# lxvm/AutoBZCore.jl

Hardware: AMD Instinct MI355X
Metric: k-point evals/sec (H(k)+eig) (higher is better)
Workload: dtype f64

## Files before the change

### autobzcore.jl_amd/_lib.py

```python
import ctypes as C
import os

import numpy as np

_HERE = os.path.dirname(os.path.abspath(__file__))
LIB_PATH = os.environ.get("ABZ_LIB") or os.path.join(_HERE, "libabzhip.so")

c_i32p = C.POINTER(C.c_int32)
c_i64p = C.POINTER(C.c_int64)
c_f64p = C.POINTER(C.c_double)
c_vpp = C.POINTER(C.c_void_p)
c_ip = C.POINTER(C.c_int)

PROTOTYPES = {
    "abz_last_error": (C.c_char_p, []),
    "abz_version": (C.c_int, []),
    "abz_device_count": (C.c_int, [c_ip]),
    "abz_ctx_create": (C.c_int, [C.c_int, c_vpp]),
    "abz_ctx_create_on_stream": (C.c_int, [C.c_int, C.c_void_p, c_vpp]),
    "abz_ctx_destroy": (C.c_int, [C.c_void_p]),
    "abz_ctx_sync": (C.c_int, [C.c_void_p]),
    "abz_prof_enable": (C.c_int, [C.c_void_p, C.c_int]),
    "abz_prof_reset": (C.c_int, [C.c_void_p]),
    "abz_prof_read": (C.c_int, [C.c_void_p, C.c_int, c_f64p, c_i64p]),
# ... 41 lines not shown
    "abz_rule_ltm_node_weights_ptr": (C.c_int, [C.c_void_p, c_vpp, c_i64p, c_ip]),
    "abz_rule_ltm_node_weights_dot": (C.c_int, [C.c_void_p, c_f64p]),
    "abz_rule_ltm_node_weights_fold": (C.c_int, [C.c_void_p, c_f64p]),
    "abz_rule_ltm_density_matrix": (C.c_int, [C.c_void_p, c_f64p]),
    "abz_rule_ltm_green_node_weights": (C.c_int, [C.c_void_p, c_f64p, C.c_int, c_f64p]),
    "abz_rule_ltm_green_node_weights_ptr": (C.c_int, [C.c_void_p, c_vpp, c_i64p, c_ip]),
    "abz_rule_ltm_green_node_weights_dot": (C.c_int, [C.c_void_p, c_f64p]),
    "abz_rule_ltm_green_node_weights_fold": (C.c_int, [C.c_void_p, c_f64p]),
    "abz_rule_ltm_green_node_weights_matrix": (C.c_int, [C.c_void_p, c_f64p]),
    "abz_mem_info": (C.c_int, [C.c_void_p, c_i64p]),
    "abz_symptr_rule": (C.c_int, [C.c_int, C.c_int, c_i32p, C.c_int, c_i64p, c_i32p, c_i64p]),
    "abz_symptr_rule_device": (C.c_int, [C.c_void_p, C.c_int, C.c_int, c_i32p, C.c_int, c_i64p, c_i32p, c_i64p]),
    "abz_contract_nodes": (C.c_int, [C.c_void_p, C.c_int, c_i64p, c_f64p, C.c_int64, c_i64p]),
    "abz_eval_line_nodes": (C.c_int, [C.c_void_p, c_i64p, c_f64p, c_f64p, C.c_int64, C.c_int, c_f64p, C.c_int,
                                      C.c_double, c_f64p]),
    "abz_release_level": (C.c_int, [C.c_void_p, C.c_int]),
    "abz_iai_solve": (C.c_int, [C.c_void_p, C.c_int, c_f64p, c_f64p, C.c_int, c_f64p, C.c_int, C.c_double, C.c_double,
                                C.c_double, C.c_int64, C.c_int64, c_f64p, c_f64p, c_i64p, c_f64p, C.c_int64, c_i64p]),
    "abz_iai_solve_many": (C.c_int, [C.c_void_p, C.c_int, c_f64p, c_f64p, C.c_int, c_f64p, C.c_int, c_f64p, C.c_int,
                                     C.c_double, C.c_double, C.c_int64, C.c_int64, c_f64p, c_f64p, c_i64p, c_f64p,
                                     C.c_int64, c_i64p]),
    "abz_iai_set_exchange": (C.c_int, [C.c_void_p, C.c_void_p, C.c_void_p, C.c_int, C.c_int]),
    "abz_gk15_nodes": (C.c_int, [C.c_double, C.c_double, c_f64p]),
    "abz_gk15_batch": (C.c_int, [c_f64p, c_f64p, C.c_int64, C.c_int, c_f64p, c_f64p]),
}

WANT_H, WANT_EIG, WANT_VEL = 1, 2, 4
WANT_H_COMPACT = 8
WANT_H_ROW_MAJOR = 16
F_ONE, F_LINEAR, F_LINEAR_X, F_DOS, F_TRGLOC, F_GLOC, F_DOS_EIG = range(7)
LIMS_CUBIC, LIMS_TETRAHEDRAL, LIMS_POLYHEDRAL, LIMS_POLYGON = 0, 1, 2, 3
K_CONTRACT, K_EVAL, K_REDUCE, K_GGR, K_EIG, K_GGRBUILD, K_LTM = range(7)
K_EVAL_FUSED = 7
LTM_DOS, LTM_STATES, LTM_STATES_CORRECTED = 0, 1, 2
LTM_A_ELEMENTS, LTM_A_ENERGY = 0, 1
LTM_A_ONE = 2
LTM_MAX_COMP = 16
LTM_EXPECT_MAX_OPS = 8
LTM_PAIRS_MAX_OPS = 4
MAX_BANDS = 64
LTM_NODEW_MAX_E = 16
LTM_GREEN_NODEW_MAX_Z = 8
PIVOT_NONE, PIVOT_PARTIAL = 0, 1
ERR_ARG, ERR_HIP, ERR_NOGPU, ERR_UNSUPPORTED, ERR_NOMEM, ERR_INTERNAL = -1, -2, -3, -4, -5, -6


EXCHANGE_FN = C.CFUNCTYPE(C.c_int, C.c_void_p, C.POINTER(C.c_double), C.c_int64)


class AbzError(RuntimeError):
    """A libabzhip call failed (ABZ_ERR_ARG is raised as ValueError = the reference's ArgumentError)."""


_lib = None


def lib():
    global _lib
    if _lib is None:
        if not os.path.exists(LIB_PATH):
            raise AbzError(f"{LIB_PATH} is missing: build it with __graft_entry__.build(); "
                           "the product has no CPU fallback")
        handle = C.CDLL(LIB_PATH)
        for name, (res, args) in PROTOTYPES.items():
            fn = getattr(handle, name)
            fn.restype = res
# ... 78 lines not shown
```

### autobzcore.jl_amd/csrc/abz_internal.h

```cpp
#pragma once
#include <hip/hip_ext.h>
#include <hip/hip_runtime.h>

#include <atomic>
#include <cstdint>
#include <cstdio>
#include <memory>
#include <string>
#include <vector>

#include "../../include/abzhip.h"
#include "dev_buf.h"
#include "ltm_block.h"
#include "plane_view.h"

namespace abz {
struct ProfScope;
struct RulePlan;

void set_error(const char* fmt, ...);
int catch_status() noexcept;

#define ABZ_CATCH_ALL \
    catch (...) { return abz::catch_status(); }
// ... 19 lines not shown
enum Switch {
    SW_POOL_MB,
    SW_DEBUG_TIMING,
    SW_EVAL_PACKED,
    SW_DOS3_SCAN,
    SW_REDUCE_ROWS,
    SW_ADAPT_PAIR,
    SW_GEN_SUM_TRI,
    SW_IPANEL_FOLD,
    SW_IPANEL_FMAC,
    SW_GGR_FUSED,
    SW_GGR_FUSE2,
    SW_GGR_UNIFORM,
    SW_IAI_SPECULATE,
    SW_IAI_PACKED,
    SW_IAI_POOL_MB,
    SW_IAI_DEVICE_INNER,
    SW_IAI_PANELS,
    SW_IAI_STATS,
    SW_HOST_THREADS,
    SW_AUTO_SWEEP_MAPPED,
    SW_LANE_KERNELS,
    SW_BIG_MFMA,
    SW_BIG_CHUNK_MB,
    SW_BIG_TRI_WAVES,
    SW_EIG_FOLD,
    SW_EIG_SPLIT,
    SW_IAI_LANES,
    SW_IAI_LANE_MIN,
    SW_CHAIN_FUSED,
    SW_EVAL_FUSED,
    SW_EVAL_PAIRS,
    SW_EVAL_MIRROR,
    SW_COUNT
};
int abz_switch(Switch s);

int stage_h2d(abz_ctx* ctx, void* dst_dev, const void* src_host, size_t bytes);
int stage_d2h(abz_ctx* ctx, void* dst_host, const void* src_dev, size_t bytes);
int mbox_reserve(abz_ctx* ctx);

int sweep_to_device(abz_ctx* ctx, const double* host, int n, const double** dev);

struct SumOut {
    double* host = nullptr;
    double* dev = nullptr;
    double2* map_dev = nullptr;
    const double2* map_host = nullptr;
};
int sum_target(abz_ctx* ctx, const SumOut& so, int64_t col0, int64_t ncols, double2** where);
int sum_deliver(abz_ctx* ctx, const SumOut& so, const double2* from, int64_t col0, int64_t ncols);

struct EnergyList {
    std::vector<int> perm;
    std::vector<double> Es, res;
    const double* dev = nullptr;
    double* out = nullptr;
    double* extra = nullptr;
    const double* res_host = nullptr;
    bool mbox = false;
    int width = 1;
    double inv_step = 0.0;
};
int energies_to_device(abz_ctx* ctx, const double* Es_host, int n, bool uniform, size_t extra, EnergyList& el, int width = 1);
int energies_deliver(abz_ctx* ctx, EnergyList& el, double* out_host);
struct SymTables;
int sym_tables_device(abz_ctx* ctx, int npt, int d, const int32_t* syms, int nsyms, SymTables& out);
void preload_symptr_code();

struct SymTables {
    int npt = 0, d = 0;
    int64_t nk = 0;
    int64_t nitems[ABZ_MAX_DIM + 1] = {0, 0, 0, 0};
    DevBuf arena;
    size_t arena_bytes = 0;
    int32_t* idx = nullptr;
    double* w = nullptr;
    int32_t* gi[ABZ_MAX_DIM + 1] = {nullptr, nullptr, nullptr, nullptr};
    int64_t* parent[ABZ_MAX_DIM + 1] = {nullptr, nullptr, nullptr, nullptr};
    int64_t* runs = nullptr;
    std::vector<int32_t> syms;
};

struct ProfSlot {
    double ms = 0.0;
    int64_t launches = 0;
    std::vector<std::pair<hipEvent_t, hipEvent_t>> pending;
};

}

struct abz_ctx {
    std::atomic<int> refs{1};
    bool closed = false;
    int device = 0;
    hipStream_t stream = nullptr;
    bool owns_stream = true;
    unsigned prof = 0;
    abz::ProfScope* prof_scope = nullptr;
    abz::ProfSlot prof_slots[ABZ_K_COUNT];
    std::vector<hipEvent_t> event_pool;
    abz::DevBuf scratch[8];
    void* pin = nullptr;
    size_t pin_cap = 0;
    std::vector<std::unique_ptr<abz::SymTables>> sym_cache;
    std::vector<std::pair<int, abz::DevBuf>> phase_cache;
    void* mbox = nullptr;
    void* mbox_dev = nullptr;
    size_t mbox_cap = 0;
};

namespace abz {
inline bool mbox_half_fits(abz_ctx* ctx, size_t bytes) { return mbox_reserve(ctx) == ABZ_OK && bytes <= ctx->mbox_cap / 2; }
template <class T>
inline T* mbox_results(abz_ctx* ctx, bool device_view) {
    return reinterpret_cast<T*>(static_cast<char*>(device_view ? ctx->mbox_dev : ctx->mbox) + ctx->mbox_cap / 2);
}
inline SumOut sum_out_mailbox(abz_ctx* ctx, double* host, size_t ncols) {
    SumOut so;
    so.host = host;
    if (mbox_half_fits(ctx, sizeof(double2) * ncols)) {
        so.map_dev = mbox_results<double2>(ctx, true);
        so.map_host = mbox_results<const double2>(ctx, false);
    }
    return so;
}
struct SeriesRule {
    int npt = 0, want = 0;
    std::vector<int32_t> syms;
    abz_rule* r = nullptr;
    uint64_t generation = 0;
    uint64_t stamp = 0;
};
// ... 130 lines not shown
int launch_contract(abz_ctx* ctx, const double2* src, int64_t src_slot_elems, const int64_t* parents,
                    int64_t per_parent, const double2* phs, double2* out, int64_t B, int64_t L, int M);

constexpr int ABZ_CONTRACT_GRID_MAXM = 16;
int launch_contract_grid(abz_ctx* ctx, const double2* src, int64_t src_slot_elems, int64_t nparents, const double2* tab,
                         double2* out, int64_t L, int M, int first, int npt, bool deriv, int gbeg, int gcnt,
                         const double2* phs_table = nullptr);
bool contract_chain_fits(int64_t L, int M3, int M2, int npt, int gcnt);
int launch_contract_chain(abz_ctx* ctx, const double2* src, const double2* phs3, const double2* phs2, double2* out,
                          int64_t L, int M3, int M2, int npt, int gbeg, int gcnt);

struct EvalSpec {
    int n;
    int M, first;
    double period;
    const double2* src;
    bool grid;
    int npt;
    int64_t nlines;
    const double2* tab;
    int64_t nk;
    const int64_t* run_start = nullptr;
    int64_t nruns = 0;
    const int64_t* parents;
    const int32_t* gi;
    const double* x;
    bool deriv;
    bool herm;
    bool packed = false;
    const double2* src2 = nullptr;
    const double2* phs2 = nullptr;
    int M2 = 0;
    bool mirror = false;
    PlaneView H;
    PlaneView E;
    PlaneView U;
};
int launch_eval(abz_ctx* ctx, const EvalSpec& es);
bool eval_packed_supported(int n, int M, int npt);
bool eval_mirror_supported(const EvalSpec& es);
bool eval_fused_supported(int n, int64_t mnn, int M2, int npt, bool pairs = false);
int launch_pack_rows(abz_ctx* ctx, int n, int M, const double2* src, int64_t nrows, double2* out);
size_t packed_row_elems(int n, int M);
int series_ensure_packed(abz_series* s);

int launch_eig_planes(abz_ctx* ctx, int n, PlaneView H, PlaneView E, PlaneView U, int64_t nk);
int launch_velocity(abz_ctx* ctx, int n, PlaneView U, PlaneView dH, PlaneView Vj, int64_t nk);

struct ReduceSpec {
    int n, d, npt;
    int integrand;
    PlaneView H;
    PlaneView E;
    int64_t nk;
    const double* w;
    const int32_t* idx;
    int64_t k_offset = 0;
    bool herm = false;
    bool pivot = false;
    double params[4];
    const double* sweep_dev;
    int n_sweep;
    double scale;
    double* tri_cache = nullptr;
    int64_t tri_nk = 0;
    int* tri_state = nullptr;
// ... 240 lines not shown
```

### autobzcore.jl_amd/csrc/api.cpp

```cpp
#include <algorithm>
#include <atomic>
#include <cstdarg>
#include <chrono>
#include <cmath>
#include <cstring>
#include <map>
#include <mutex>
#include <numeric>
#include <thread>

#include "abz_internal.h"

namespace abz {

static thread_local std::string g_err;

void set_error(const char* fmt, ...) {
    char buf[1024];
    va_list ap;
    va_start(ap, fmt);
    vsnprintf(buf, sizeof(buf), fmt, ap);
    va_end(ap);
    g_err = buf;
}
// ... 31 lines not shown
const SwitchDef g_switches[SW_COUNT] = {
    {"ABZ_POOL_MB", 4096, "MB of freed device blocks the caching allocator keeps per device"},
    {"ABZ_DEBUG_TIMING", 0, "1: wall time of the rule-build phases on stderr (synchronises after each)"},
    {"ABZ_EVAL_PACKED", 1, "0: full-grid chains on plain coefficient sets instead of packed Hermitian sets"},
    {"ABZ_DOS3_SCAN", 1, "0: 3-band DOS sweeps through the generic reduce_kernel"},
    {"ABZ_REDUCE_ROWS", 0, "> 0: rows of blocks a sweep is split over in the scan kernels"},
    {"ABZ_ADAPT_PAIR", 1, "0: one-lane adaptive step in the device-side GK loops"},
    {"ABZ_GEN_SUM_TRI", 1, "0: 5...16-band sweeps with one inversion per swept value"},
    {"ABZ_IPANEL_FOLD", 1, "0: 16-lane panel kernel on the unfolded series"},
    {"ABZ_IPANEL_FMAC", 1, "0: 16-lane panel kernel with separate pivot-row broadcasts"},
    {"ABZ_GGR_FUSED", 1, "0: GGR build by eigenvectors + one velocity launch per variable"},
    {"ABZ_GGR_FUSE2", 1, "0: fused GGR build reads level-1 families instead of contracting variable 2 itself"},
    {"ABZ_GGR_UNIFORM", 1, "0: GGR scans search the energy window even in equispaced lists"},
    {"ABZ_IAI_SPECULATE", 1, "0: nested IAI driver requests one panel per integral and round"},
    {"ABZ_IAI_PACKED", 1, "0: IAI chains on plain coefficient sets"},
    {"ABZ_IAI_POOL_MB", 0, "> 0: MB per chunk of level sets in the IAI driver (default: sized from free memory)"},
    {"ABZ_IAI_DEVICE_INNER", 1, "0: innermost GK loops driven from the host, one launch per round"},
    {"ABZ_IAI_PANELS", 1, "0: the level above the innermost one ships nodes instead of panels (GK rule of that level on the host)"},
    {"ABZ_IAI_STATS", 0, "1: per-solve statistics of the IAI driver on stderr"},
    {"ABZ_HOST_THREADS", 8, "host threads for the per-integral bookkeeping of IAI sweeps (capped at half the cores)"},
    {"ABZ_AUTO_SWEEP_MAPPED", 1, "0: abz_autoptr_solve* uploads its swept values instead of letting the kernels read the pinned host copy"},
    {"ABZ_LANE_KERNELS", 1, "0: 5...8-band rule builds / store-free sums on full grids through the 8-lane row kernels (test: same values)"},
    {"ABZ_BIG_MFMA", 0, "1: 33...64 bands: the level-1 evaluation of full grid lines as a real GEMM on v_mfma_f64_16x16x4_f64 (test: same values)"},
    {"ABZ_BIG_CHUNK_MB", 0, "33...64 bands: MB of scratch for the matrices of a chunk of nodes (0: 256, GGR builds 2048; tests set 1 to walk many chunks)"},
    {"ABZ_BIG_TRI_WAVES", 0, "33...64 bands: waves per node of the Householder tridiagonalisation (1, 2, 4: the same reflectors, another summation order; 0: two up to 44 bands, one up to 48, four above)"},
    {"ABZ_EIG_FOLD", 1, "0: 5...16-band rule builds evaluate the full level-1 series of a Hermitian model instead of the folded one"},
    {"ABZ_EIG_SPLIT", 1, "0: eigenvalues of 5...16-band rules by bisection inside the grid kernel instead of the per-lane QR kernel"},
    {"ABZ_IAI_LANES", 4, "lanes (host thread + stream each) a sweep of independent IAI solves is split over; 1: off"},
    {"ABZ_IAI_LANE_MIN", 16, "solves per lane below which a sweep is not split further"},
    {"ABZ_CHAIN_FUSED", 1, "0: 3-D full-grid chains contract variables 3 and 2 in two launches instead of contract_chain_kernel"},
    {"ABZ_EVAL_FUSED", 1, "0: 3-D full-grid rules (n <= 4) build level-1 sets with contract_chain_kernel instead of contracting variable 2 inside the grid kernel"},
    {"ABZ_EVAL_PAIRS", 1, "fused grid kernel, one grid line per half-wave: 1 where it takes fewer lane-rounds per line (Hermitian series), 0 never, 2 wherever supported (tests: same values)"},
    {"ABZ_EVAL_MIRROR", 1, "3-D full-grid rules (n <= 4) of a real Hermitian series evaluate the planes k3 <= npt/2 and store H(-k) = conj H(k) beside them: 1 where the launch writes at most 600 MB, 0 never (every plane evaluated), 2 wherever supported"},
};
}

int abz_switch(Switch s) {
    const char* e = getenv(g_switches[s].name);
    return (e && *e) ? atoi(e) : g_switches[s].dflt;
}

namespace {
struct Block {
    void* p;
    size_t cap;
    int device;
};
std::mutex g_pool_mutex;
std::vector<Block> g_pool;
size_t g_pool_bytes = 0;
std::atomic<int64_t> g_live_bytes{0};
std::atomic<int64_t> g_live_blocks{0};
size_t pool_limit() {
    static const size_t lim = (size_t)std::max(0, abz_switch(SW_POOL_MB)) << 20;
    return lim;
}
void pool_flush(int device) {
    for (size_t i = 0; i < g_pool.size();) {
        if (g_pool[i].device == device) {
            (void)hipFree(g_pool[i].p);
            g_pool_bytes -= g_pool[i].cap;
            g_pool[i] = g_pool.back();
            g_pool.pop_back();
        } else {
            ++i;
        }
// ... 244 lines not shown
}

ProfScope::ProfScope(abz_ctx* c, int kernel_id) : ctx(c), id(kernel_id) {
    if (!(ctx->prof & (1u << id))) return;
    auto get = [&]() {
        hipEvent_t e = nullptr;
        if (!ctx->event_pool.empty()) {
            e = ctx->event_pool.back();
            ctx->event_pool.pop_back();
        } else if (hipEventCreateWithFlags(&e, hipEventDisableSystemFence) != hipSuccess) {
            e = nullptr;
        }
        return e;
    };
    e0 = get();
    e1 = get();
    if (!e0 || !e1) return;
    outer = ctx->prof_scope;
    ctx->prof_scope = this;
}

ProfScope::~ProfScope() {
    if (!(ctx->prof & (1u << id))) return;
    if (e0 && e1) ctx->prof_scope = outer;
    if (!e0 || !e1 || !started) {
        if (e0) ctx->event_pool.push_back(e0);
        if (e1) ctx->event_pool.push_back(e1);
        return;
    }
    ctx->prof_slots[id].pending.emplace_back(e0, e1);
}

int prof_collect(abz_ctx* ctx) {
    for (int i = 0; i < ABZ_K_COUNT; ++i) {
        auto& sl = ctx->prof_slots[i];
        for (auto& pr : sl.pending) {
            ABZ_HIP(hipEventSynchronize(pr.second));
            float ms = 0.f;
            ABZ_HIP(hipEventElapsedTime(&ms, pr.first, pr.second));
            sl.ms += ms;
            sl.launches += 1;
            ctx->event_pool.push_back(pr.first);
            ctx->event_pool.push_back(pr.second);
        }
        sl.pending.clear();
    }
    return ABZ_OK;
}

template <class T>
static int upload(abz_ctx* ctx, DevBuf& buf, const T* host, size_t count) {
    int rc = buf.reserve(sizeof(T) * std::max<size_t>(count, 1));
    if (rc) return rc;
    if (count) return stage_h2d(ctx, buf.p, host, sizeof(T) * count);
    return ABZ_OK;
}

struct Plan {
    int d = 0;
    bool full = false;
    bool coords = false;
    int npt = 0;
    int outer0 = 0, outer_n = 0;
    int64_t nk = 0;
    int64_t nitems[ABZ_MAX_DIM + 1] = {0, 0, 0, 0};
    std::vector<int32_t> gi[ABZ_MAX_DIM + 1];
    std::vector<double> xs[ABZ_MAX_DIM + 1];
// ... 333 lines not shown
    ABZ_REQUIRE(ctx, "null ctx");
    ctx->prof = on == 0 ? 0u : (on == 1 ? 0xffffffffu : ((unsigned)on >> 1));
    return ABZ_OK;
} ABZ_CATCH_ALL

int abz_mem_info(abz_ctx* ctx, int64_t* info) try {
    ABZ_REQUIRE(info, "abz_mem_info: null info");
    {
        std::lock_guard<std::mutex> lk(g_pool_mutex);
        info[1] = (int64_t)g_pool_bytes;
    }
    info[0] = g_live_bytes.load();
    info[2] = 0;
    info[3] = 0;
    info[4] = g_live_blocks.load();
    if (ctx) {
        for (const auto& b : ctx->scratch) info[2] += (int64_t)b.cap;
        info[3] = (int64_t)ctx->pin_cap;
    }
    return ABZ_OK;
} ABZ_CATCH_ALL

int abz_prof_reset(abz_ctx* ctx) try {
    ABZ_REQUIRE(ctx, "null ctx");
    int rc = prof_collect(ctx);
    for (auto& sl : ctx->prof_slots) {
        sl.ms = 0;
        sl.launches = 0;
    }
    return rc;
} ABZ_CATCH_ALL

int abz_prof_read(abz_ctx* ctx, int kernel_id, double* total_ms, int64_t* launches) try {
    ABZ_REQUIRE(ctx && kernel_id >= 0 && kernel_id < ABZ_K_COUNT, "bad profile slot");
    int rc = prof_collect(ctx);
    if (rc) return rc;
    if (total_ms) *total_ms = ctx->prof_slots[kernel_id].ms;
    if (launches) *launches = ctx->prof_slots[kernel_id].launches;
    return ABZ_OK;
} ABZ_CATCH_ALL

static bool detect_hermitian(const abz_series* s, const double* coef_reim);
static bool detect_real(const abz_series* s, const double* coef_reim);

int abz_series_create(abz_ctx* ctx, const double* coef_reim, int d, const int32_t* dims, const int32_t* first,
                      const double* period, int n, abz_series** out) try {
    ABZ_REQUIRE(ctx && coef_reim && dims && first && period && out, "abz_series_create: null argument");
    ABZ_REQUIRE(!ctx->closed, "abz_series_create: the context was destroyed");
    ABZ_REQUIRE(d >= 1 && d <= ABZ_MAX_DIM, "series dimension d = %d not in 1..%d", d, ABZ_MAX_DIM);
    ABZ_REQUIRE(n >= 1 && n <= ABZ_MAX_BANDS, "n = %d bands not in 1..%d", n, ABZ_MAX_BANDS);
    *out = nullptr;
    ABZ_HIP(hipSetDevice(ctx->device));
    std::unique_ptr<abz_series> s(new abz_series());
    s->ctx = ctx;
    s->d = d;
    s->n = n;
    for (int j = 0; j < d; ++j) {
        ABZ_REQUIRE(dims[j] >= 1 && period[j] > 0, "dims[%d] = %d / period = %g invalid", j, dims[j], period[j]);
        s->dims[j] = dims[j];
        s->first[j] = first[j];
        s->period[j] = period[j];
    }
    const size_t bytes = sizeof(double2) * (size_t)s->elems(d);
    if (s->coef.alloc(bytes)) return ABZ_ERR_NOMEM;
    hipError_t e = hipMemcpy(s->coef.p, coef_reim, bytes, hipMemcpyHostToDevice);
    if (e != hipSuccess) {
        set_error("coefficient upload failed: %s", hipGetErrorString(e));
// ... 293 lines not shown
                        const double2* level2 = nullptr) -> int {
        EvalSpec es;
        es.n = n;
        es.M = s->dims[0];
        es.first = s->first[0];
        es.period = s->period[0];
        es.src = level1;
        if (level2) {
            es.src2 = level2;
            es.phs2 = rp->pd.phg[1].as<double2>();
            es.M2 = s->dims[1];
        }
        es.grid = r->full;
        es.npt = r->npt;
        es.nlines = r->full ? (d == 1 ? 1 : plan.nitems[1]) : 0;
        es.tab = tab;
        es.nk = r->nk;
        es.parents = r->full ? nullptr : rp->pd.parent[0].as<int64_t>();
        es.gi = r->full ? nullptr : rp->pd.gi[0].as<int32_t>();
        if (!r->full && plan.nruns > 0 && !plan.coords) {
            es.run_start = rp->pd.runs.as<int64_t>();
            es.nruns = plan.nruns;
        }
        es.x = nullptr;
        es.deriv = deriv;
        es.herm = s->hermitian;
        es.packed = packed_chain && !deriv && !Uout.base;
        const int sw_mirror = abz_switch(SW_EVAL_MIRROR);
        const PlaneView& pv = Hout.base ? Hout : Eout;
        const double out_bytes = 8.0 * ((Hout.base ? (Hout.compact ? 1.0 : 2.0) * n * n : 0.0) + (Eout.base ? (double)n : 0.0)) *
                                 (double)pv.row * (double)es.nlines;
        es.mirror = s->hermitian && s->real_coef && r->full && d == 3 && plan.outer_n == r->npt && !deriv && !Uout.base &&
                    !(r->want & ABZ_WANT_VEL) && (sw_mirror >= 2 || (sw_mirror == 1 && out_bytes <= 600e6));
        es.H = Hout;
        es.E = Eout;
        es.U = Uout;
        return launch_eval(ctx, es);
    };
    const double2* level1 = nullptr;
    int rc;
    const int64_t line_elems = packed_chain ? (int64_t)packed_row_elems(n, s->dims[0]) : (int64_t)s->dims[0] * n * n;
    const bool ref_layout_large = s->hermitian && r->H.base && !r->H.compact && r->npt > 64;
    const bool eval_fused = r->full && d == 3 && n <= 4 && !(r->want & ABZ_WANT_VEL) && !Uv.base && rp->pd.phg[2].p && rp->pd.phg[1].p &&
                            !ref_layout_large &&
                            abz_switch(SW_CHAIN_FUSED) && abz_switch(SW_EVAL_FUSED) &&
                            contract_chain_fits(line_elems, s->dims[2], s->dims[1], r->npt, plan.outer_n) &&
                            eval_fused_supported(n, line_elems, s->dims[1], r->npt);
    if (eval_fused) {
        const double2* level2 = nullptr;
        if ((rc = build_chain(s, plan, rp->pd, tab, 0, &level2, 2, nullptr, packed_chain))) return rc;
        return run_eval(nullptr, false, r->H, r->E, PlaneView(), level2);
    }
    if ((rc = build_chain(s, plan, rp->pd, tab, 0, &level1, 1, nullptr, packed_chain))) return rc;
    if ((rc = run_eval(level1, false, r->H, vel_done ? PlaneView() : r->E, Uv))) return rc;
    if ((r->want & ABZ_WANT_VEL) && !vel_done) {
        for (int j = 1; j <= d; ++j) {
            if (j >= 2)
                if ((rc = build_chain(s, plan, rp->pd, tab, j, &level1))) return rc;
            if ((rc = run_eval(level1, j == 1, Dv, PlaneView(), PlaneView()))) return rc;
            PlaneView Vj = r->V;
            Vj.base += (int64_t)(j - 1) * n * Vj.pitch;
            if ((rc = launch_velocity(ctx, n, Uv, Dv, Vj, r->nk))) return rc;
        }
    }
    return ABZ_OK;
}
// ... 876 lines not shown
```

### autobzcore.jl_amd/csrc/kernels.hip

```cpp
#include "abz_internal.h"
#include "device_math.h"
#include "gk15.h"
#include "inner_adapt.h"
#include "packed_herm.h"

#include <cmath>
#include <cstring>
#include <type_traits>
#include <utility>
#include <cstdlib>

namespace abz {

static inline int64_t cdiv(int64_t a, int64_t b) { return (a + b - 1) / b; }

struct cplx_pod {
    double x, y;
};
typedef const cplx_pod __attribute__((address_space(4))) * cptr_t;
__device__ __forceinline__ cptr_t as_const(const double2* p) {
    return (cptr_t)(unsigned long long)p;
}

struct PhaseArgs {
// ... 771 lines not shown
__device__ __forceinline__ void load_line_phases(cptr_t p, LinePhases& ph) {
#pragma unroll
    for (int m = 0; m < ABZ_CONTRACT_GRID_MAXM; ++m) {
        ph.x[m] = p[m].x;
        ph.y[m] = p[m].y;
    }
}

template <int M2>
__device__ __forceinline__ void contract_line(const double2* s2, const LinePhases& ph, double2* dst, int MNN, int lane) {
    for (int l = lane; l < MNN; l += 64) {
        double ar = 0.0, ai = 0.0;
#pragma unroll
        for (int m = 0; m < M2; ++m) {
            const double2 c = s2[m * MNN + l];
            ar = fma(c.x, ph.x[m], ar);
            ar = fma(-c.y, ph.y[m], ar);
            ai = fma(c.x, ph.y[m], ai);
            ai = fma(c.y, ph.x[m], ai);
        }
        dst[l] = make_double2(ar, ai);
    }
}

__device__ __forceinline__ void contract_line_m(int M2, const double2* s2, const LinePhases& ph, double2* dst, int MNN, int lane) {
#define CL(MM) case MM: contract_line<MM>(s2, ph, dst, MNN, lane); break;
    switch (M2) {
        CL(1) CL(2) CL(3) CL(4) CL(5) CL(6) CL(7) CL(8) CL(9) CL(10) CL(11) CL(12) CL(13) CL(14) CL(15) CL(16)
        default: break;
    }
#undef CL
}

template <int N, int KPL, bool HERM, bool VEC, int OCC, bool PK = false, bool FUSE = false, bool PAIR = false, int KT = KPL, bool MIR = false>
__global__ __launch_bounds__(256, OCC) void eval_grid_kernel(EvalArgs a) {
    static_assert(!MIR || (HERM && !VEC), "mirrored launches: values and eigenvalues of a Hermitian series");
    static_assert(FUSE || !PAIR, "the pair mapping exists in the fused instance only");
    static_assert(KT >= 1 && KT <= KPL && (PAIR || KT == KPL), "a shorter last pass exists in the pair mapping only");
    constexpr int LPU = PAIR ? 2 : 1;
    extern __shared__ double2 lds_c[];
    const int wave = __builtin_amdgcn_readfirstlane(threadIdx.x >> 6), lane = threadIdx.x & 63;
    const int MNN = PK ? Pk<N>::size((a.M - 1) / 2) : a.M * N * N;
    auto stage = [&](double2 c, int idx) -> double2 {
        if (!a.deriv) return c;
        const double f = 6.283185307179586476925286766559 * (double)(a.first + idx / (N * N));
        return make_double2(-f * c.y, f * c.x);
    };
    double2* const mybuf = lds_c + (size_t)wave * 2 * LPU * MNN;
    int fm = a.first % a.npt;
    if (fm < 0) fm += a.npt;
    constexpr int LW = 64 / LPU;
    const int npass = (a.npt + LW * KPL - 1) / (LW * KPL);
    double2* const tab_l = lds_c + (size_t)4 * 2 * LPU * MNN;
    if constexpr (FUSE) {
        static_assert(!VEC, "the fused instance stores values and eigenvalues only");
        const int k3 = blockIdx.y, seg = blockIdx.x;
        const int mk3 = (MIR && k3 != 0 && 2 * k3 != a.npt) ? a.npt - k3 : -1;
        const int L2 = a.M2 * MNN;
        const double2* __restrict__ src2 = a.src2 + (int64_t)k3 * L2;
        double2* const s2 = tab_l + a.npt;
        const int kstride = 4 * a.bpk;
        int k2 = LPU * (4 * seg + wave);
        LinePhases ph;
        load_line_phases(as_const(a.phs2 + (int64_t)(k2 < a.npt ? k2 : 0) * a.M2), ph);
        {
            const int it = threadIdx.x;
            double2 vt = a.tab[min(it, a.npt - 1)];
            double2 v[4];
#pragma unroll
            for (int j = 0; j < 4; ++j) v[j] = src2[min(it + 256 * j, L2 - 1)];
            asm volatile("" : "+v"(vt.x), "+v"(vt.y));
#pragma unroll
            for (int j = 0; j < 4; ++j) asm volatile("" : "+v"(v[j].x), "+v"(v[j].y));
            if (it < a.npt) tab_l[it] = vt;
#pragma unroll
            for (int j = 0; j < 4; ++j)
                if (it + 256 * j < L2) s2[it + 256 * j] = v[j];
            for (int i = it + 256; i < a.npt; i += 256) tab_l[i] = a.tab[i];
            for (int i = it + 4 * 256; i < L2; i += 256) s2[i] = src2[i];
        }
        __syncthreads();
        if (k2 >= a.npt) return;
        contract_line_m(a.M2, s2, ph, mybuf, MNN, lane);
        if constexpr (PAIR) {
            const int half = lane >> 5, col = lane & 31;
            load_line_phases(as_const(a.phs2 + (int64_t)min(k2 + 1, a.npt - 1) * a.M2), ph);
            contract_line_m(a.M2, s2, ph, mybuf + MNN, MNN, lane);
            int iz0[KPL], iw0[KPL], izt[KT], iwt[KT];
#pragma unroll
            for (int j = 0; j < KPL; ++j) {
                const int i1 = col + 32 * j;
                iz0[j] = i1 < a.npt ? i1 : 0;
                iw0[j] = (int)(((unsigned)fm * (unsigned)iz0[j]) % (unsigned)a.npt);
                if (j < KT) {
                    izt[j] = iz0[j];
                    iwt[j] = iw0[j];
                }
            }
            const int off_h = half * (int)a.H.tile, off_e = half * (int)a.E.tile;
            int cur = 0, pass = 0;
            while (k2 < a.npt) {
                const bool last_pass = pass + 1 >= npass;
                const int nk2 = last_pass ? k2 + 2 * kstride : k2;
                const bool contract_next = last_pass && nk2 < a.npt;
                wave_lds_sync();
                auto mid_fn = [&]() __attribute__((always_inline)) {
                    if (contract_next) {
                        int ln = lane;
                        asm volatile("" : "+v"(ln));
                        double2* const dst = mybuf + (size_t)(cur ^ 1) * 2 * MNN;
                        load_line_phases(as_const(a.phs2 + (int64_t)nk2 * a.M2), ph);
                        contract_line_m(a.M2, s2, ph, dst, MNN, ln);
                        load_line_phases(as_const(a.phs2 + (int64_t)min(nk2 + 1, a.npt - 1) * a.M2), ph);
                        contract_line_m(a.M2, s2, ph, dst + MNN, MNN, ln);
                    }
                };
                const double2* const c1 = mybuf + (size_t)(2 * cur + half) * MNN;
                const int64_t line = (int64_t)k3 * a.npt + k2;
                const bool on = half == 0 || k2 + 1 < a.npt;
                MirrorTo mt;
// ... 272 lines not shown
                if (cost < best - 1e-12) {
                    best = cost;
                    kpl = k;
                }
            }
        }
        const size_t lds = sizeof(double2) * (4 * 2 * (size_t)mnn + (size_t)a.npt);
        if (es.src2) {
            if (es.deriv || es.U.base || !eval_fused_supported(es.n, mnn, es.M2, es.npt) || es.nlines % es.npt != 0 ||
                es.nlines / es.npt > 65535) {
                set_error("eval: fused contraction unsupported (n = %d, %d numbers per line, M2 = %d, npt = %d)", es.n, mnn, es.M2, es.npt);
                return ABZ_ERR_UNSUPPORTED;
            }
            const int64_t gcnt = es.nlines / es.npt;
            a.mirror = eval_mirror_supported(es) ? 1 : 0;
            const unsigned grows = a.mirror ? (unsigned)(es.npt / 2 + 1) : (unsigned)gcnt;
            a.src2 = es.src2;
            a.phs2 = es.phs2;
            a.M2 = es.M2;
            if (ctx->prof & (1u << ABZ_K_EVAL_FUSED)) ctx->prof_slots[ABZ_K_EVAL_FUSED].launches += 1;
            a.bpk = (int)std::max<int64_t>(1, std::min<int64_t>(cdiv(es.npt, 4), cdiv(blocks, gcnt)));
            a.bpk = (int)cdiv(es.npt, 4 * cdiv(es.npt, 4 * a.bpk));
            const size_t flds = lds + sizeof(double2) * (size_t)es.M2 * mnn;
            const int sw_pairs = abz_switch(SW_EVAL_PAIRS);
            const int rounds = (int)cdiv(es.npt, 32);
            const bool pairs = sw_pairs != 0 && eval_fused_supported(es.n, mnn, es.M2, es.npt, true) && es.H.tile < INT32_MAX &&
                               es.E.tile < INT32_MAX && (sw_pairs >= 2 || (a.herm && rounds < 2 * cdiv(es.npt, 64 * kpl) * kpl));
            if (pairs) {
                const int kp = es.n < 4 ? 3 : (a.herm ? 2 : 1);
                const int kt = rounds - (int)(cdiv(rounds, kp) - 1) * kp;
                const int64_t npairs = cdiv(es.npt, 2);
                a.bpk = (int)std::max<int64_t>(1, std::min<int64_t>(cdiv(npairs, 4), cdiv(blocks, gcnt)));
                a.bpk = (int)cdiv(npairs, 4 * cdiv(npairs, 4 * a.bpk));
                const size_t plds = flds + sizeof(double2) * 4 * 2 * (size_t)mnn;
                const dim3 grid((unsigned)a.bpk, grows);
#define LKP(NN, KT)                                                                                                          \
    {                                                                                                                        \
        constexpr int OO = NN == 3 ? 3 : 2;                                                                                  \
        constexpr int KH = NN < 4 ? 3 : 2, KG = NN < 4 ? 3 : 1;                                                \
        if (a.herm)                                                                                                          \
            with_flags(a.pk != 0, a.mirror != 0, [&](auto pk, auto mir) {                                                    \
                launch(ctx, eval_grid_kernel<NN, KH, true, false, OO, pk(), true, true, KT <= KH ? KT : KH, mir()>, grid, dim3(256), plds, a); \
            });                                                                                                              \
        else                                                                                                                 \
            launch(ctx, eval_grid_kernel<NN, KG, false, false, 2, false, true, true, KT <= KG ? KT : KG>, grid, dim3(256), plds, a); \
    }
#define FN(NN)                     \
    switch (kt) {                  \
        case 1: LKP(NN, 1) break;  \
        case 2: LKP(NN, 2) break;  \
        default: LKP(NN, 3) break; \
    }
                ABZ_DISPATCH_N(es.n, FN)
#undef FN
#undef LKP
            } else {
#define LK(NN, KK)                                                                                                                         \
    {                                                                                                                                      \
        constexpr int OO = NN == 3 ? 3 : 2;                                                                                                \
        if (a.herm)                                                                                                                        \
            with_flags(a.pk != 0, a.mirror != 0, [&](auto pk, auto mir) {                                                                  \
                launch(ctx, eval_grid_kernel<NN, KK, true, false, OO, pk(), true, false, KK, mir()>, dim3((unsigned)a.bpk, grows), dim3(256), flds, a); \
            });                                                                                                                            \
        else                                                                                                                               \
            launch(ctx, eval_grid_kernel<NN, KK, false, false, 2, false, true>, dim3((unsigned)a.bpk, grows), dim3(256), flds, a); \
    }
#define FN(NN)                    \
    switch (kpl) {                \
        case 1: LK(NN, 1) break;  \
        case 2: LK(NN, 2) break;  \
        default: LK(NN, 3) break; \
    }
            ABZ_DISPATCH_N(es.n, FN)
#undef FN
#undef LK
// ... 1852 lines not shown
```

### include/abzhip.h

```cpp
#ifndef ABZHIP_H
#define ABZHIP_H

#include <stddef.h>
#include <stdint.h>

#ifdef __cplusplus
extern "C" {
#endif

#define ABZ_VERSION 502

#define ABZ_OK 0
#define ABZ_ERR_ARG (-1)
#define ABZ_ERR_HIP (-2)
#define ABZ_ERR_NOGPU (-3)
#define ABZ_ERR_UNSUPPORTED (-4)
#define ABZ_ERR_NOMEM (-5)
#define ABZ_ERR_INTERNAL (-6)

#define ABZ_MAX_DIM 3
#define ABZ_MAX_BANDS 64

typedef struct abz_ctx abz_ctx;
typedef struct abz_series abz_series;
typedef struct abz_rule abz_rule;

#define ABZ_WANT_H 1
#define ABZ_WANT_EIG 2
#define ABZ_WANT_VEL 4
#define ABZ_WANT_H_COMPACT 8
#define ABZ_WANT_H_ROW_MAJOR 16

#define ABZ_F_ONE 0
#define ABZ_F_LINEAR 1
#define ABZ_F_LINEAR_X 2
#define ABZ_F_DOS 3
#define ABZ_F_TRGLOC 4
#define ABZ_F_GLOC 5
#define ABZ_F_DOS_EIG 6

#define ABZ_LIMS_CUBIC 0
#define ABZ_LIMS_TETRAHEDRAL 1
#define ABZ_LIMS_POLYHEDRAL 2
#define ABZ_LIMS_POLYGON 3

#define ABZ_K_CONTRACT 0
#define ABZ_K_EVAL 1
#define ABZ_K_REDUCE 2
#define ABZ_K_GGR 3
#define ABZ_K_EIG 4
#define ABZ_K_GGRBUILD 5
#define ABZ_K_LTM 6
#define ABZ_K_EVAL_FUSED 7
#define ABZ_K_COUNT 8

int abz_mem_info(abz_ctx* ctx, int64_t* info);

const char* abz_last_error(void);
int abz_version(void);
int abz_device_count(int* n);
int abz_ctx_create(int device, abz_ctx** out);
int abz_ctx_create_on_stream(int device, void* hip_stream, abz_ctx** out);
int abz_ctx_destroy(abz_ctx* ctx);
int abz_ctx_sync(abz_ctx* ctx);
int abz_prof_enable(abz_ctx* ctx, int on);
int abz_prof_reset(abz_ctx* ctx);
int abz_prof_read(abz_ctx* ctx, int kernel_id, double* total_ms, int64_t* launches);

int abz_series_create(abz_ctx* ctx, const double* coef_reim, int d, const int32_t* dims,
                      const int32_t* first, const double* period, int n, abz_series** out);
int abz_series_destroy(abz_series* s);
int abz_series_update(abz_series* s, const double* coef_reim);
#define ABZ_PIVOT_NONE 0
#define ABZ_PIVOT_PARTIAL 1
int abz_series_set_pivoting(abz_series* s, int mode);
int abz_series_get_pivoting(const abz_series* s, int* mode);

int abz_eval_nodes(abz_series* s, const double* k, int64_t nk, int want, double* H_out,
                   double* eig_out);

int abz_ptr_rule_build(abz_series* s, int npt, int64_t nirr, const int32_t* irr_idx,
                       const int64_t* wsym, int want, abz_rule** out);

int abz_ptr_rule_build_sym(abz_series* s, int npt, const int32_t* syms, int nsyms, int want,
                           abz_rule** out);

int abz_ptr_rule_build_slab(abz_series* s, int npt, int outer_begin, int outer_end, int want,
// ... 108 lines not shown
```

Baseline: 50.22 billion.

## Map one pass of each line pair per wave in fused Hermitian grid eval

Adds a variant of the fused pair-mapped grid kernel in which each wave handles a single pass of a line pair instead of all passes, multiplying the block count by the pass count. The per-wave LDS buffer is halved, since each wave contracts its line pair once and evaluates only its slice. The aim is more parallelism and occupancy when there are only 2 or 4 passes per line. The cost is that each line's contraction is recomputed once per pass. A selection rule plus an env switch enable it, and a profiling slot is added.

Measured after the change: 55.15 billion, median of 6. 9.8% higher.

```diff
diff --git a/autobzcore.jl_amd/_lib.py b/autobzcore.jl_amd/_lib.py
--- a/autobzcore.jl_amd/_lib.py
+++ b/autobzcore.jl_amd/_lib.py
@@ -97,6 +97,7 @@
 LIMS_CUBIC, LIMS_TETRAHEDRAL, LIMS_POLYHEDRAL, LIMS_POLYGON = 0, 1, 2, 3
 K_CONTRACT, K_EVAL, K_REDUCE, K_GGR, K_EIG, K_GGRBUILD, K_LTM = range(7)
 K_EVAL_FUSED = 7
+K_EVAL_PASSWAVE = 8
 LTM_DOS, LTM_STATES, LTM_STATES_CORRECTED = 0, 1, 2
 LTM_A_ELEMENTS, LTM_A_ENERGY = 0, 1
 LTM_A_ONE = 2
diff --git a/autobzcore.jl_amd/csrc/abz_internal.h b/autobzcore.jl_amd/csrc/abz_internal.h
--- a/autobzcore.jl_amd/csrc/abz_internal.h
+++ b/autobzcore.jl_amd/csrc/abz_internal.h
@@ -75,6 +75,7 @@
     SW_EVAL_FUSED,
     SW_EVAL_PAIRS,
     SW_EVAL_MIRROR,
+    SW_EVAL_PASSWAVE,
     SW_COUNT
 };
 int abz_switch(Switch s);
@@ -141,7 +142,7 @@
     bool owns_stream = true;
     unsigned prof = 0;
     abz::ProfScope* prof_scope = nullptr;
-    abz::ProfSlot prof_slots[ABZ_K_COUNT];
+    abz::ProfSlot prof_slots[ABZ_K_SLOTS];
     std::vector<hipEvent_t> event_pool;
     abz::DevBuf scratch[8];
     void* pin = nullptr;
@@ -338,6 +339,7 @@
     const double2* phs2 = nullptr;
     int M2 = 0;
     bool mirror = false;
+    bool passwave = false;
     PlaneView H;
     PlaneView E;
     PlaneView U;
diff --git a/autobzcore.jl_amd/csrc/api.cpp b/autobzcore.jl_amd/csrc/api.cpp
--- a/autobzcore.jl_amd/csrc/api.cpp
+++ b/autobzcore.jl_amd/csrc/api.cpp
@@ -87,6 +87,7 @@
     {"ABZ_EVAL_FUSED", 1, "0: 3-D full-grid rules (n <= 4) build level-1 sets with contract_chain_kernel instead of contracting variable 2 inside the grid kernel"},
     {"ABZ_EVAL_PAIRS", 1, "fused grid kernel, one grid line per half-wave: 1 where it takes fewer lane-rounds per line (Hermitian series), 0 never, 2 wherever supported (tests: same values)"},
     {"ABZ_EVAL_MIRROR", 1, "3-D full-grid rules (n <= 4) of a real Hermitian series evaluate the planes k3 <= npt/2 and store H(-k) = conj H(k) beside them: 1 where the launch writes at most 600 MB, 0 never (every plane evaluated), 2 wherever supported"},
+    {"ABZ_EVAL_PASSWAVE", 1, "fused pair mapping of Hermitian series, pairs of 2 or 4 passes: one pass of a pair per wave instead of a pair per wave: 1 by the selection rule, 0 never, 2 wherever supported (tests: same values)"},
 };
 }
 
@@ -397,7 +398,7 @@
 }
 
 int prof_collect(abz_ctx* ctx) {
-    for (int i = 0; i < ABZ_K_COUNT; ++i) {
+    for (int i = 0; i < ABZ_K_SLOTS; ++i) {
         auto& sl = ctx->prof_slots[i];
         for (auto& pr : sl.pending) {
             ABZ_HIP(hipEventSynchronize(pr.second));
@@ -797,7 +798,7 @@
 } ABZ_CATCH_ALL
 
 int abz_prof_read(abz_ctx* ctx, int kernel_id, double* total_ms, int64_t* launches) try {
-    ABZ_REQUIRE(ctx && kernel_id >= 0 && kernel_id < ABZ_K_COUNT, "bad profile slot");
+    ABZ_REQUIRE(ctx && kernel_id >= 0 && kernel_id < ABZ_K_SLOTS, "bad profile slot");
     int rc = prof_collect(ctx);
     if (rc) return rc;
     if (total_ms) *total_ms = ctx->prof_slots[kernel_id].ms;
@@ -1157,6 +1158,9 @@
                                  (double)pv.row * (double)es.nlines;
         es.mirror = s->hermitian && s->real_coef && r->full && d == 3 && plan.outer_n == r->npt && !deriv && !Uout.base &&
                     !(r->want & ABZ_WANT_VEL) && (sw_mirror >= 2 || (sw_mirror == 1 && out_bytes <= 600e6));
+        const int sw_passwave = abz_switch(SW_EVAL_PASSWAVE);
+        const int rounds = (r->npt + 31) / 32, per_pass = n < 4 ? 3 : 2;
+        es.passwave = sw_passwave >= 2 || (sw_passwave == 1 && rounds > per_pass && rounds <= 2 * per_pass);
         es.H = Hout;
         es.E = Eout;
         es.U = Uout;
diff --git a/autobzcore.jl_amd/csrc/kernels.hip b/autobzcore.jl_amd/csrc/kernels.hip
--- a/autobzcore.jl_amd/csrc/kernels.hip
+++ b/autobzcore.jl_amd/csrc/kernels.hip
@@ -827,12 +827,15 @@
 #undef CL
 }
 
-template <int N, int KPL, bool HERM, bool VEC, int OCC, bool PK = false, bool FUSE = false, bool PAIR = false, int KT = KPL, bool MIR = false>
+template <int N, int KPL, bool HERM, bool VEC, int OCC, bool PK = false, bool FUSE = false, bool PAIR = false, int KT = KPL, bool MIR = false,
+          bool PW = false>
 __global__ __launch_bounds__(256, OCC) void eval_grid_kernel(EvalArgs a) {
     static_assert(!MIR || (HERM && !VEC), "mirrored launches: values and eigenvalues of a Hermitian series");
     static_assert(FUSE || !PAIR, "the pair mapping exists in the fused instance only");
     static_assert(KT >= 1 && KT <= KPL && (PAIR || KT == KPL), "a shorter last pass exists in the pair mapping only");
+    static_assert(!PW || (PAIR && HERM), "one pass per wave exists in the pair mapping of Hermitian series only");
     constexpr int LPU = PAIR ? 2 : 1;
+    constexpr int NBUF = PW ? 1 : 2;
     extern __shared__ double2 lds_c[];
     const int wave = __builtin_amdgcn_readfirstlane(threadIdx.x >> 6), lane = threadIdx.x & 63;
     const int MNN = PK ? Pk<N>::size((a.M - 1) / 2) : a.M * N * N;
@@ -841,12 +844,12 @@
         const double f = 6.283185307179586476925286766559 * (double)(a.first + idx / (N * N));
         return make_double2(-f * c.y, f * c.x);
     };
-    double2* const mybuf = lds_c + (size_t)wave * 2 * LPU * MNN;
+    double2* const mybuf = lds_c + (size_t)wave * NBUF * LPU * MNN;
     int fm = a.first % a.npt;
     if (fm < 0) fm += a.npt;
     constexpr int LW = 64 / LPU;
     const int npass = (a.npt + LW * KPL - 1) / (LW * KPL);
-    double2* const tab_l = lds_c + (size_t)4 * 2 * LPU * MNN;
+    double2* const tab_l = lds_c + (size_t)4 * NBUF * LPU * MNN;
     if constexpr (FUSE) {
         static_assert(!VEC, "the fused instance stores values and eigenvalues only");
         const int k3 = blockIdx.y, seg = blockIdx.x;
@@ -856,6 +859,12 @@
         double2* const s2 = tab_l + a.npt;
         const int kstride = 4 * a.bpk;
         int k2 = LPU * (4 * seg + wave);
+        int pw_pass = 0;
+        if constexpr (PW) {
+            const int u = 4 * seg + wave;
+            pw_pass = u & (npass - 1);
+            k2 = 2 * (u >> (npass == 4 ? 2 : 1));
+        }
         LinePhases ph;
         load_line_phases(as_const(a.phs2 + (int64_t)(k2 < a.npt ? k2 : 0) * a.M2), ph);
         {
@@ -881,6 +890,27 @@
             const int half = lane >> 5, col = lane & 31;
             load_line_phases(as_const(a.phs2 + (int64_t)min(k2 + 1, a.npt - 1) * a.M2), ph);
             contract_line_m(a.M2, s2, ph, mybuf + MNN, MNN, lane);
+            if constexpr (PW) {
+                const int seeds[KPL] = {}, seeds_t[KT] = {};
+                const int64_t line = (int64_t)k3 * a.npt + k2;
+                MirrorTo mt;
+                if (mk3 >= 0) {
+                    mt.line = (int64_t)mk3 * a.npt;
+                    mt.t0 = k2 ? a.npt - k2 : 0;
+                    mt.t1 = k2 + 1 < a.npt ? a.npt - k2 - 1 : 0;
+                }
+                auto no_mid = []() {};
+                wave_lds_sync();
+                if (KT == KPL || pw_pass + 1 < npass)
+                    eval_unit<N, KPL, HERM, VEC, decltype(no_mid)&, PK, 32>(a, mybuf + (size_t)half * MNN, tab_l, fm, seeds, seeds, 2, pw_pass * (32 * KPL),
+                                                                            col, line, no_mid, half * (int)a.H.tile, half * (int)a.E.tile,
+                                                                            half == 0 || k2 + 1 < a.npt, mt);
+                else
+                    eval_unit<N, KT, HERM, VEC, decltype(no_mid)&, PK, 32>(a, mybuf + (size_t)half * MNN, tab_l, fm, seeds_t, seeds_t, 2, pw_pass * (32 * KPL),
+                                                                           col, line, no_mid, half * (int)a.H.tile, half * (int)a.E.tile,
+                                                                           half == 0 || k2 + 1 < a.npt, mt);
+                return;
+            }
             int iz0[KPL], iw0[KPL], izt[KT], iwt[KT];
 #pragma unroll
             for (int j = 0; j < KPL; ++j) {
@@ -1219,7 +1249,14 @@
                 const int64_t npairs = cdiv(es.npt, 2);
                 a.bpk = (int)std::max<int64_t>(1, std::min<int64_t>(cdiv(npairs, 4), cdiv(blocks, gcnt)));
                 a.bpk = (int)cdiv(npairs, 4 * cdiv(npairs, 4 * a.bpk));
-                const size_t plds = flds + sizeof(double2) * 4 * 2 * (size_t)mnn;
+                size_t plds = flds + sizeof(double2) * 4 * 2 * (size_t)mnn;
+                const int npass = (int)cdiv(rounds, kp);
+                const bool passwave = es.passwave && a.herm && (npass == 2 || npass == 4);
+                if (passwave) {
+                    a.bpk = (int)cdiv(npairs * npass, 4);
+                    plds = flds;
+                    if (ctx->prof & (1u << ABZ_K_EVAL_PASSWAVE)) ctx->prof_slots[ABZ_K_EVAL_PASSWAVE].launches += 1;
+                }
                 const dim3 grid((unsigned)a.bpk, grows);
 #define LKP(NN, KT)                                                                                                          \
     {                                                                                                                        \
@@ -1227,7 +1264,10 @@
         constexpr int KH = NN < 4 ? 3 : 2, KG = NN < 4 ? 3 : 1;                                                \
         if (a.herm)                                                                                                          \
             with_flags(a.pk != 0, a.mirror != 0, [&](auto pk, auto mir) {                                                    \
-                launch(ctx, eval_grid_kernel<NN, KH, true, false, OO, pk(), true, true, KT <= KH ? KT : KH, mir()>, grid, dim3(256), plds, a); \
+                if (passwave)                                                                                                \
+                    launch(ctx, eval_grid_kernel<NN, KH, true, false, OO, pk(), true, true, KT <= KH ? KT : KH, mir(), true>, grid, dim3(256), plds, a); \
+                else                                                                                                         \
+                    launch(ctx, eval_grid_kernel<NN, KH, true, false, OO, pk(), true, true, KT <= KH ? KT : KH, mir()>, grid, dim3(256), plds, a); \
             });                                                                                                              \
         else                                                                                                                 \
             launch(ctx, eval_grid_kernel<NN, KG, false, false, 2, false, true, true, KT <= KG ? KT : KG>, grid, dim3(256), plds, a); \
diff --git a/include/abzhip.h b/include/abzhip.h
--- a/include/abzhip.h
+++ b/include/abzhip.h
@@ -53,6 +53,8 @@
 #define ABZ_K_LTM 6
 #define ABZ_K_EVAL_FUSED 7
 #define ABZ_K_COUNT 8
+#define ABZ_K_EVAL_PASSWAVE 8
+#define ABZ_K_SLOTS 9
 
 int abz_mem_info(abz_ctx* ctx, int64_t* info);
 
```
